# ethnhe/FFB6D

Measured on AMD Instinct MI355X. Metric: RGB-D frames/sec fwd (480x640, N=12288, bs=8), higher is better.
Workload: dtype f32; 1 GPU; FFB6D forward incl. on-device 22-call KNN index pyramid; bs=8/GPU, N=12288 pts, 480x640 RGB-D, 22 classes, fp32, eval; global_batch=8, n_points=12288, index_dtype=int64, layout=pm, parallelism=dp1 (independent batches, one process per GPU, no process group)

## Files before the change

### ffb6d_amd/_lib.py

```python
import ctypes
import os

from . import build as _build

_c = ctypes
_vp, _i64, _i32, _sz = _c.c_void_p, _c.c_int64, _c.c_int, _c.c_size_t

SIGNATURES = {
    "ffb6d_last_error": (_c.c_char_p, []),
    "ffb6d_abi_version": (_c.c_int, []),
    "cpp_knn": (None, [_vp, _sz, _sz, _vp, _sz, _sz, _vp]),
    "cpp_knn_omp": (None, [_vp, _sz, _sz, _vp, _sz, _sz, _vp]),
    "cpp_knn_batch": (None, [_vp, _sz, _sz, _sz, _vp, _sz, _sz, _vp]),
    "cpp_knn_batch_omp": (None, [_vp, _sz, _sz, _sz, _vp, _sz, _sz, _vp]),
    "cpp_knn_batch_distance_pick": (None, [_vp, _sz, _sz, _sz, _vp, _sz, _sz, _vp]),
    "cpp_knn_batch_distance_pick_omp": (None, [_vp, _sz, _sz, _sz, _vp, _sz, _sz, _vp]),
    "ffb6d_knn_workspace_bytes": (_sz, [_i64, _i64, _i64, _i32]),
    "ffb6d_knn_batch_device": (_i32, [_vp, _vp, _i64, _i64, _i64, _i32, _vp, _vp, _vp, _vp, _sz, _vp]),
    "ffb6d_knn_prepared_bytes": (_sz, [_i64, _i64]),
    "ffb6d_knn_prepare_workspace_bytes": (_sz, [_i64, _i64]),
    "ffb6d_knn_prepare": (_i32, [_vp, _i64, _i64, _vp, _sz, _vp, _sz, _vp]),
    "ffb6d_knn_prepare_multi_workspace_bytes": (_sz, [_i32, _vp, _i64]),
    "ffb6d_knn_prepare_multi": (_i32, [_i32, _vp, _vp, _i64, _vp, _vp, _vp, _sz, _vp]),
    "ffb6d_knn_search_multi": (_i32, [_i32, _vp, _i64, _vp]),
    "ffb6d_knn_search_prepared": (_i32, [_vp, _vp, _vp, _i64, _i64, _i64, _i32, _vp, _vp, _vp, _vp]),
    "ffb6d_knn_set_pair_counter": (_i32, [_vp]),
    "ffb6d_knn_uses_pruning": (_i32, [_i64, _i64, _i64, _i32]),
    "ffb6d_random_sample_f32": (_i32, [_vp, _vp, _i32, _vp, _vp, _i64, _i64, _i64, _i64, _i32, _vp]),
    "ffb6d_random_sample_bwd_f32": (_i32, [_vp, _vp, _vp, _i64, _i64, _i64, _i64, _vp]),
    "ffb6d_nearest_interpolation_f32": (_i32, [_vp, _vp, _i32, _vp, _i64, _i64, _i64, _i64, _vp]),
    "ffb6d_nearest_interpolation_bwd_f32": (_i32, [_vp, _vp, _i32, _vp, _i64, _i64, _i64, _i64, _vp]),
    "ffb6d_gather_neighbour_f32": (_i32, [_vp, _vp, _i32, _vp, _i64, _i64, _i64, _i64, _i32, _vp]),
    "ffb6d_gather_neighbour_bwd_f32": (_i32, [_vp, _vp, _i32, _vp, _i64, _i64, _i64, _i64, _i32, _vp]),
    "ffb6d_relative_pos_encoding_f32": (_i32, [_vp, _vp, _i32, _vp, _i64, _i64, _i32, _vp]),
    "ffb6d_att_pool_f32": (_i32, [_vp, _vp, _vp, _i64, _i64, _i64, _i32, _vp]),
    "ffb6d_relative_pos_encoding_cm_f32": (_i32, [_vp, _vp, _i32, _vp, _i64, _i64, _i32, _vp]),
    "ffb6d_att_pool_bwd_f32": (_i32, [_vp, _vp, _vp, _vp, _vp, _i64, _i64, _i64, _i32, _vp]),
    "ffb6d_mlp_pm_f32": (_i32, [_vp, _vp, _vp, _i64, _i64, _vp, _i64, _vp, _i64, _i64, _vp, _i64, _vp, _i64, _i32, _i64, _vp,
                                _i64, _i64, _i64, _i32, _i32, _vp]),
    "ffb6d_mlp_pm_tile": (_i32, [_i64, _i64, _i64, _i32]),
    "ffb6d_mlp_pm_choice": (_i32, [_i64, _i64, _i64, _i64, _i32, _i32, _i32]),
    "ffb6d_mlp_pm_seq_plan": (_i32, [_i64, _i64]),
    "ffb6d_mlp_pm_batched_f32": (_i32, [_vp, _i64, _i64, _vp, _i64, _i64, _vp, _i64, _i64, _i64, _i32, _vp]),
    "ffb6d_mlp_pm_split_w": (_i32, [_vp, _vp, _i64, _vp]),
    "ffb6d_mlp_pm_split_f32": (_i32, [_vp, _vp, _vp, _i64, _i64, _vp, _i64, _vp, _i64, _i64, _vp, _i64, _vp, _i64, _i32, _i64, _vp,
                                      _i64, _i64, _i64, _i32, _i32, _vp]),
    "ffb6d_mlp_pm_split_batched_f32": (_i32, [_vp, _i64, _i64, _vp, _i64, _i64, _vp, _i64, _i64, _i64, _vp]),
    "ffb6d_wino_input_f32": (_i32, [_vp, _vp, _i64, _i64, _i64, _i64, _i64, _vp]),
    "ffb6d_wino_output_f32": (_i32, [_vp, _vp, _vp, _vp, _vp, _vp, _vp, _i64, _i64, _i64, _i64, _i64, _i32, _c.c_float, _vp]),
    "ffb6d_wino4_input_f32": (_i32, [_vp, _vp, _i64, _i64, _i64, _i64, _i64, _vp]),
    "ffb6d_wino4_output_f32": (_i32, [_vp, _vp, _vp, _vp, _vp, _vp, _vp, _i64, _i64, _i64, _i64, _i64, _i32, _c.c_float, _vp]),
    "ffb6d_wino4_conv_f32": (_i32, [_vp, _vp, _vp, _vp, _vp, _vp, _vp, _vp, _i64, _i64, _i64, _i64, _i64, _i32, _c.c_float, _i32, _vp]),
    "ffb6d_wino4_conv_form": (_i32, [_i64, _i64]),
    "ffb6d_mlp_pm_set_big_form": (None, [_i32]),
    "ffb6d_mlp_pm_set_seq_lin": (None, [_i32]),
    "ffb6d_att_pool_pm_f32": (_i32, [_vp, _vp, _i64, _i64, _vp, _i32, _vp, _i64, _i64, _vp, _i64, _i64, _i64, _i32, _vp]),
    "ffb6d_mlp_pm_bf16": (_i32, [_vp, _vp, _vp, _i64, _i64, _vp, _i64, _vp, _i64, _i64, _vp, _i64, _vp, _i64, _i32, _i64, _vp,
                                 _i64, _i64, _i64, _i32, _i32, _vp]),
    "ffb6d_att_pool_pm_bf16": (_i32, [_vp, _vp, _i64, _i64, _vp, _i32, _vp, _i64, _i64, _vp, _i64, _i64, _i64, _i32, _vp]),
    "ffb6d_random_sample_pm": (_i32, [_i32, _vp, _vp, _i32, _vp, _i64, _i64, _i64, _i64, _i32, _vp]),
    "ffb6d_gather_rows_pm": (_i32, [_i32, _vp, _vp, _i32, _vp, _i64, _i64, _i64, _i64, _vp]),
    "ffb6d_relative_pos_encoding_pm": (_i32, [_i32, _vp, _vp, _i32, _vp, _i64, _i64, _i32, _vp]),
    "ffb6d_affine_act_pm": (_i32, [_i32, _vp, _vp, _vp, _vp, _vp, _vp, _vp, _i64, _i64, _i32, _c.c_float, _vp]),
    "ffb6d_affine_relu_maxpool_pm": (_i32, [_i32, _vp, _vp, _vp, _vp, _i64, _i64, _i64, _i64, _vp]),
    "ffb6d_bilinear_resize_pm": (_i32, [_i32, _vp, _vp, _i64, _i64, _i64, _i64, _i64, _i64, _i32, _vp]),
    "ffb6d_mlp_chain3_pm_f32": (_i32, [_vp, _i64, _vp, _vp, _i32, _vp, _vp, _i32, _vp, _vp, _i32, _vp, _i64, _i64, _i64, _vp]),
    "ffb6d_mlp_chain3_pm_bf16": (_i32, [_vp, _i64, _vp, _vp, _i32, _vp, _vp, _i32, _vp, _vp, _i32, _vp, _i64, _i64, _i64, _vp]),
    "ffb6d_upsampled_patch_rows_pm": (_i32, [_i32, _vp, _vp, _i32, _vp, _i64, _i64, _i64, _i64, _i64, _i64, _i64, _vp]),
    "ffb6d_posenc_mlp_pm": (_i32, [_i32, _vp, _vp, _i32, _vp, _i64, _vp, _i32, _vp, _i64, _i64, _i32, _i64, _vp]),
    "ffb6d_lfa_pm": (_i32, [_i32, _i32, _vp, _i64, _vp, _i32, _vp, _i64, _vp, _i64, _vp, _i32, _vp, _vp, _i32, _vp, _vp, _vp, _i32, _vp, _i64,
                            _i64, _i64, _i32, _i64, _i32, _vp]),
    "ffb6d_lfa_pm_choice": (_i32, [_i64, _i64, _i32]),
    "ffb6d_bilinear_bwd_pm": (_i32, [_i32, _vp, _vp, _i64, _i64, _i64, _i64, _i64, _i64, _vp]),
    "ffb6d_prelu_fwd": (_i32, [_i32, _vp, _vp, _vp, _i64, _vp]),
    "ffb6d_prelu_bwd": (_i32, [_i32, _vp, _vp, _vp, _vp, _vp, _i64, _vp]),
    "ffb6d_gather_sum_rows": (_i32, [_i32, _vp, _i64, _vp, _vp, _vp, _i64, _i64, _vp]),
    "ffb6d_random_sample_rows_bwd": (_i32, [_i32, _vp, _vp, _i32, _vp, _i64, _vp, _i64, _i64, _i64, _i64, _i32, _vp]),
    "ffb6d_att_pool_rows": (_i32, [_i32, _vp, _i64, _vp, _i64, _vp, _i64, _i32, _i64, _vp]),
    "ffb6d_att_pool_rows_bwd": (_i32, [_i32, _vp, _i64, _vp, _i64, _vp, _i64, _vp, _vp, _i64, _i32, _i64, _vp]),
    "ffb6d_log_softmax_rows": (_i32, [_i32, _vp, _vp, _i64, _i64, _vp]),
    "ffb6d_log_softmax_rows_bwd": (_i32, [_i32, _vp, _vp, _vp, _i64, _i64, _vp]),
    "ffb6d_upconv_combine_pm": (_i32, [_i32, _vp, _vp, _c.c_float, _vp, _i64, _i64, _i64, _i64, _i64, _i64, _vp]),
    "ffb6d_upconv_set_form": (None, [_i32]),
    "ffb6d_pose_set_fit_form": (None, [_i32]),
    "ffb6d_pose_set_fit_spread": (None, [_i32]),
    "ffb6d_pose_set_big_form": (None, [_i32]),
    "ffb6d_psp_pool_pm_workspace_bytes": (_sz, [_i64, _i64, _i64, _vp, _i32]),
    "ffb6d_psp_pool_pm": (_i32, [_i32, _vp, _vp, _i64, _i64, _i64, _i64, _vp, _i32, _vp, _sz, _vp]),
    "ffb6d_psp_prior_sum_pm": (_i32, [_i32, _vp, _vp, _i64, _i64, _i64, _i64, _vp, _i32, _vp]),
    "ffb6d_depth_to_cloud_f32": (_i32, [_vp, _vp, _c.c_float, _vp, _i64, _i64, _i64, _vp]),
    "ffb6d_pyramid_sets_f32": (_i32, [_vp, _i64, _i64, _i64, _i64, _i64, _i32, _vp, _vp, _vp, _vp, _i64, _i64, _i32, _vp, _vp, _vp]),
    "ffb6d_sample_points_workspace_bytes": (_sz, [_i64, _i64, _i64]),
    "ffb6d_sample_points_f32": (_i32, [_vp, _c.c_float, _vp, _vp, _i32, _vp, _c.c_uint64, _vp, _vp, _vp, _vp, _i64, _i64, _i64,
                                       _i64, _vp, _sz, _vp]),
    "ffb6d_depth_normal": (_i32, [_vp, _i32, _c.c_double, _c.c_double, _i32, _i32, _i32, _i32, _vp, _i64, _i64, _i64, _vp]),
    "ffb6d_fill_missing_workspace_bytes": (_sz, [_i64, _i64, _i64]),
    "ffb6d_fill_missing_f32": (_i32, [_vp, _c.c_double, _c.c_double, _c.c_float, _vp, _i64, _i64, _i64, _vp, _sz, _vp]),
    "ffb6d_check_index_range": (_i32, [_vp, _i32, _i64, _i64, _vp, _vp]),
    "ffb6d_vote_sets_f32": (_i32, [_vp, _vp, _vp, _i32, _vp, _vp, _vp, _i32, _i32, _i32, _i32, _i64, _vp, _vp, _vp]),
    "ffb6d_mean_shift_workspace_bytes": (_sz, [_i32, _i64]),
    "ffb6d_mean_shift_f32": (_i32, [_vp, _vp, _i32, _i32, _i64, _i64, _c.c_float, _i32, _i32, _vp, _vp, _vp, _vp, _vp,
                                    _sz, _vp]),
    "ffb6d_mean_shift_multi_workspace_bytes": (_sz, [_i32, _i64]),
    "ffb6d_mean_shift_multi_f32": (_i32, [_vp, _vp, _i32, _i32, _i64, _i64, _c.c_float, _i32, _i32, _i32, _i32, _vp, _vp, _vp, _vp,
                                          _vp, _vp, _sz, _vp]),
    "ffb6d_pose_set_converged_out": (None, [_vp]),
    "ffb6d_set_clusters_to_points": (_i32, [_vp, _vp, _vp, _vp, _i32, _i64, _i32, _vp, _vp]),
    "ffb6d_vote_sets_inst_f32": (_i32, [_vp, _vp, _vp, _i32, _vp, _vp, _vp, _vp, _i32, _i32, _i32, _i32, _i64, _vp, _vp, _vp]),
    "ffb6d_set_labels_to_points": (_i32, [_vp, _vp, _vp, _vp, _i32, _i64, _i32, _vp, _vp]),
    "ffb6d_refine_mask_by_center": (_i32, [_vp, _vp, _vp, _i32, _vp, _vp, _vp, _vp, _i32, _i32, _vp, _vp]),
    "ffb6d_best_fit_transform_f32": (_i32, [_vp, _vp, _i32, _i32, _vp, _vp]),
    "ffb6d_pose_add_adds_workspace_bytes": (_sz, [_i32, _i64]),
    "ffb6d_pose_add_adds_f32": (_i32, [_vp, _vp, _i32, _vp, _vp, _vp, _i32, _vp, _vp, _vp, _sz, _vp]),
    "ffb6d_icp_prepared_bytes": (_sz, [_i64, _i32]),
    "ffb6d_icp_prepare": (_i32, [_vp, _vp, _i32, _i64, _vp, _sz, _vp]),
    "ffb6d_icp_workspace_bytes": (_sz, [_i32, _i64]),
    "ffb6d_icp_set_form": (None, [_i32]),
# ... 135 lines not shown
```

### ffb6d_amd/forward_pm.py

```python
import torch
import torch.nn.functional as F

from . import _lib, ops, ops_pm, pyramid


def cached(mod, name, sources, build):
    key = tuple((t._version, t.data_ptr(), t.device) for t in sources)
    store = mod.__dict__.setdefault("_pm_cache", {})
    hit = store.get(name)
    if hit is None or hit[0] != key:
        with torch.no_grad():
            hit = (key, build())
        store[name] = hit
    return hit[1]


def _pad_k(w, k_to):
    if w.shape[1] == k_to:
        return w.contiguous()
    out = w.new_zeros(w.shape[0], k_to)
    out[:, :w.shape[1]] = w
    return out


# ... 215 lines not shown
        return False
    cout, cin = c.weight.shape[:2]
    if cin < TRUNK_WINOGRAD_MIN_CIN or cin < 128 or cin % 32 or cout % 4:
        return False
    B, H, W, _ = x.shape
    if m is None:
        m = wino_variant(B, H, W)
    planes, Tp = (m + 2) ** 2, (ops_pm.wino4_tiles if m == 4 else ops_pm.wino_tiles)(B, H, W)[1]
    lim = (1 << 31) - (1 << 20)
    return planes * (Tp + 256) * max(cin, cout) * 4 < lim and B * H * W * max(cin, cout) * 4 < lim and planes * cout * cin * 4 < lim


def conv_wino(x, c, scale, shift, residual=None, res_affine=None, m=None):
    if m is None:
        m = wino_variant(*x.shape[:3])
    x = x if x.is_contiguous() else x.contiguous()
    if m == 4:
        v, u = ops_pm.wino4_input(x), wino4_weights(c)
        if gemm_split_takes(v.shape[0] * v.shape[1], u.shape[1], u.shape[2]):
            mm = ops_pm.mlp_batched(v, u, tile_hint=ops_pm.SPLIT_FORM, w_split=wino4_split_weights(c))
        else:
            mm = ops_pm.mlp_batched(v, u)
        return ops_pm.wino4_output(mm, x.shape[:3], scale, shift, act=ops.ACT_RELU, residual=residual, res_affine=res_affine)
    if m != 2:
        raise ValueError(f"conv_wino: m must be 2, 4 or None, got {m}")
    u = wino_weights(c)
    v = ops_pm.wino_input(x)
    mm = ops_pm.mlp_batched(v, u)
    return ops_pm.wino_output(mm, x.shape[:3], scale, shift, act=ops.ACT_RELU, residual=residual, res_affine=res_affine)


TRUNK_WINOGRAD_FUSED = True
TRUNK_WINOGRAD_FUSED_WIDTHS = frozenset({(64, 64), (128, 128), (128, 256)})


def wino_fused_ok(c, x):
    if not (TRUNK_WINOGRAD and TRUNK_WINOGRAD_FUSED) or x.dtype != torch.float32 or c.weight.dtype != torch.float32:
        return False
    if (c.kernel_size, c.stride, c.padding, c.dilation, c.groups) != ((3, 3), (1, 1), (1, 1), (1, 1), 1) or c.bias is not None \
            or c.padding_mode != "zeros":
        return False
    cout, cin = c.weight.shape[:2]
    if (cin, cout) not in TRUNK_WINOGRAD_FUSED_WIDTHS or cin not in ops_pm.WINO4_CONV_CIN or cout not in ops_pm.WINO4_CONV_COUT:
        return False
    B, H, W, _ = x.shape
    return B * H * W * max(cin, cout) * 4 < (1 << 31) - (1 << 20)


def conv_wino_fused(x, c, scale, shift, residual=None, res_affine=None):
    x = x if x.is_contiguous() else x.contiguous()
    return ops_pm.wino4_conv(x, wino4_weights(c), scale, shift, act=ops.ACT_RELU, residual=residual, res_affine=res_affine)


def trunk_conv_form(c, x):
    if wino_fused_ok(c, x):
        return "fused"
    return "wino" if wino_ok(c, x) else "miopen"


def res_block(rb, x):
    form1 = trunk_conv_form(rb.conv1, x)
    if form1 == "fused":
        y = conv_wino_fused(x, rb.conv1, *ops.bn_fold(rb.bn1))
    elif form1 == "wino":
        y = conv_wino(x, rb.conv1, *ops.bn_fold(rb.bn1))
    else:
        y = ops_pm.affine_act_(conv(x, rb.conv1), *ops.bn_fold(rb.bn1), act=ops.ACT_RELU)
    form2 = trunk_conv_form(rb.conv2, y)
    if form2 == "miopen":
        y = conv(y, rb.conv2)
    res, res_affine = x, None
    if rb.downsample is not None:
        res, res_affine = conv(x, rb.downsample[0]), ops.bn_fold(rb.downsample[1])
    if form2 == "fused":
        return conv_wino_fused(y, rb.conv2, *ops.bn_fold(rb.bn2), residual=res, res_affine=res_affine)
    if form2 == "wino":
        return conv_wino(y, rb.conv2, *ops.bn_fold(rb.bn2), residual=res, res_affine=res_affine)
    return ops_pm.affine_act_(y, *ops.bn_fold(rb.bn2), act=ops.ACT_RELU, residual=res, res_affine=res_affine)


def pyramid_pooling(pp, x):
    B, h, w_, C = x.shape
    sizes = [st[0].output_size[0] for st in pp.stages]
    bw = pp.bottleneck.weight

    def build():
        ch = pp.stages[0][1].weight.shape[0]
        wb = bw.detach().reshape(bw.shape[0], -1)
        prods = [(wb[:, i * ch:(i + 1) * ch] @ st[1].weight.detach().reshape(ch, ch)).contiguous()
                 for i, st in enumerate(pp.stages)]
        return prods, wb[:, len(pp.stages) * ch:].contiguous()
    prods, wx = cached(pp, "fold", [bw] + [st[1].weight for st in pp.stages], build)
    pooled = ops_pm.psp_pool(x, sizes)
    zs, off = [], 0
    for s, wl in zip(sizes, prods):
        zs.append(ops_pm.mlp(pooled[:, off:off + s * s].contiguous(), wl, role="cnn"))
        off += s * s
    prior = ops_pm.psp_prior_sum(torch.cat(zs, dim=1), sizes, (h, w_), dtype=x.dtype)
    wx = cached(pp, "wx%s" % x.dtype, [bw], lambda: wx.to(x.dtype))
    return mlp_long(pp, "wx", [bw], x, wx, pp.bottleneck.bias.detach().float(), ops.ACT_RELU, add=prior, role="cnn")


UPCONV_FOLD = "auto"
UPCONV_FOLD_BF16 = True


# ... 171 lines not shown

def forward(net, inputs, end_points, two_streams=True, taps=None):
    dev = inputs['rgb'].device
    dt = torch.bfloat16 if getattr(net, "precision", "fp32") == "bf16" else torch.float32
    ops_pm.MLP_SEQ_FORM = GEMM_SEQ_FORM
    ops_pm.MLP_BIG_FORM = GEMM_BIG_FORM
    ops_pm.MLP_SEQ_LIN = (2 if GEMM_SEQ_LIN_ONE else 1) if GEMM_SEQ_LIN else 0
    main = torch.cuda.current_stream(dev)
    side = net._side_stream(dev) if two_streams else main
    if two_streams:
        side.wait_stream(main)

    lazy = 'cld_nei_idx0' not in inputs
    if lazy:
        inputs = StreamedPyramid(net, inputs, main, side)

    def need(i, up=False):
        if lazy:
            (inputs.up_level if up else inputs.level)(i, side)
            if not two_streams:
                return
            (inputs.up_level if up else inputs.level)(i, main)

    def need_nearest():
        if lazy:
            inputs.nearest(side)
            if two_streams:
                inputs.nearest(main)

    def on_side():
        return torch.cuda.stream(side)

    probe = getattr(net, "_stall_probe", None)

    def handover(t, producer, consumer, tag=None):
        if producer is not consumer:
            ev = torch.cuda.Event()
            ev.record(producer)
            if probe is not None:
                a = torch.cuda.Event(enable_timing=True)
                a.record(consumer)
            consumer.wait_event(ev)
            if probe is not None:
                b = torch.cuda.Event(enable_timing=True)
                b.record(consumer)
                probe.append((tag, a, b))
            t.record_stream(consumer)
        return t

    def fuse(i, pre_p2r, fuse_p2r, pre_r2p, fuse_r2p, rgb0, p0, p2r_idx, r2p_idx):
        st = ("ds%d" if pre_p2r is net.ds_fuse_p2r_pre_layers else "up%d") % i
        return fusion_step(pre_p2r[i], fuse_p2r[i], pre_r2p[i], fuse_r2p[i], rgb0, p0, p2r_idx, r2p_idx, main, side, handover, st)

    rgb = inputs['rgb'].to(dt).contiguous(memory_format=torch.channels_last).permute(0, 2, 3, 1)
    pool = net.cnn_pre_stages[3]
    if STEM_FUSED and (pool.kernel_size, pool.stride, pool.padding, pool.dilation, pool.ceil_mode) == (3, 2, 1, 1, False):
        rgb_emb = ops_pm.affine_relu_maxpool(conv(rgb, net.cnn_pre_stages[0]), *ops.bn_fold(net.cnn_pre_stages[1]))
    else:
        y = ops_pm.affine_act_(conv(rgb, net.cnn_pre_stages[0]), *ops.bn_fold(net.cnn_pre_stages[1]), act=ops.ACT_RELU)
        rgb_emb = pool(y.permute(0, 3, 1, 2)).permute(0, 2, 3, 1)
    with on_side():
        raw = inputs['cld_rgb_nrm']
        x0 = torch.zeros(raw.shape[0], raw.shape[2], (raw.shape[1] + 15) // 16 * 16, dtype=dt, device=dev)
        x0[..., :raw.shape[1]] = raw.transpose(1, 2)
        c_pre = net.rndla_pre_stages.conv.weight.shape[0]
        p_emb = torch.zeros(raw.shape[0], raw.shape[2], (c_pre + 15) // 16 * 16, dtype=dt, device=dev)
        mlp(net.rndla_pre_stages, x0, pad_k=x0.shape[-1], out=p_emb[..., :c_pre])

    ds_emb = []
    for i in range(4):
        rgb0 = cnn_stage(net.cnn_ds_stages[i], rgb_emb)
        need(i)
        with on_side():
            xyz = inputs['cld_xyz%d' % i]
            if LFA_FUSED:
                xyz = inputs.xyz_table(i) if lazy else ops_pm.xyz_table(xyz)
            f_enc = dilated_res_block(net.rndla_ds_stages[i], p_emb, xyz, inputs['cld_nei_idx%d' % i])
            p0 = ops_pm.random_sample(f_enc, inputs['cld_sub_idx%d' % i])
        if i == 0:
            ds_emb.append(f_enc)
        need_nearest()
        rgb_emb, p_emb = fuse(i, net.ds_fuse_p2r_pre_layers, net.ds_fuse_p2r_fuse_layers, net.ds_fuse_r2p_pre_layers,
                              net.ds_fuse_r2p_fuse_layers, rgb0, p0, inputs['p2r_ds_nei_idx%d' % i],
                              inputs['r2p_ds_nei_idx%d' % i])
        ds_emb.append(p_emb)
        if taps is not None:
            torch.cuda.synchronize(dev)
            taps['rgb_emb_ds%d' % i], taps['p_emb_ds%d' % i] = rgb_emb.permute(0, 3, 1, 2).float(), p_emb.transpose(1, 2).unsqueeze(3).float()

    n_up = len(net.rndla_up_stages)
    for i in range(n_up - 1):
        rgb0 = cnn_stage(net.cnn_up_stages[i], rgb_emb)
        need(i, up=True)
        need_nearest()
        with on_side():
            p0 = decode(net.rndla_up_stages[i], ds_emb[-i - 2], p_emb, inputs['cld_interp_idx%d' % (n_up - i - 1)])
        rgb_emb, p_emb = fuse(i, net.up_fuse_p2r_pre_layers, net.up_fuse_p2r_fuse_layers, net.up_fuse_r2p_pre_layers,
                              net.up_fuse_r2p_fuse_layers, rgb0, p0, inputs['p2r_up_nei_idx%d' % i],
                              inputs['r2p_up_nei_idx%d' % i])
        if taps is not None:
            torch.cuda.synchronize(dev)
            taps['rgb_emb_up%d' % i], taps['p_emb_up%d' % i] = rgb_emb.permute(0, 3, 1, 2).float(), p_emb.transpose(1, 2).unsqueeze(3).float()
    B = rgb_emb.shape[0]
    choose = inputs['choose'].reshape(B, -1)
    img = last_stage_at_chosen(net.cnn_up_stages[n_up - 1], rgb_emb, choose) if LAST_STAGE_AT_CHOSEN else None
    if img is not None:
        choose = None
    else:
        rgb_emb = cnn_stage(net.cnn_up_stages[n_up - 1], rgb_emb)
        img = rgb_emb.view(B, -1, rgb_emb.shape[-1])
    with on_side():
        p_emb = decode(net.rndla_up_stages[n_up - 1], ds_emb[0], p_emb, inputs['cld_interp_idx0'])
    handover(p_emb, side, main, "main waits for the last decoder")
# ... 57 lines not shown
```

### ffb6d_amd/ops_pm.py

```python
import torch

from . import _lib
from .ops import ACT_LEAKY, ACT_NONE, ACT_RELU, _idx, _need_gpu, _stream


def _dt(*ts):
    dts = {t.dtype for t in ts if t is not None}
    if len(dts) != 1 or next(iter(dts)) not in (torch.float32, torch.bfloat16):
        raise TypeError(f"row operands must all be float32 or all bfloat16, got {sorted(map(str, dts))}")
    return 1 if next(iter(dts)) == torch.bfloat16 else 0


def rows_view(x):
    C = x.shape[-1]
    x2 = x.reshape(-1, C)
    if x2.stride(1) != 1 or x2.data_ptr() % 16 or (x2.shape[0] > 1 and (x2.stride(0) * x2.element_size()) % 16):
        x2 = x2.contiguous()
    return x2, (x2.stride(0) if x2.shape[0] > 1 else C)


ACT_LOG_SOFTMAX = 3
MLP_SEQ_FORM = True
MLP_BIG_FORM = True
MLP_SEQ_LIN = 0
# ... 450 lines not shown
    ib = bits // 8
    ref_bytes = (12 * B * N + ib * B * N * K + 40 * B * N * K if mode == 1 else 0) + (esz * B * N * h + ib * B * N * K + esz * B * N * K * h) \
        + (2 * esz * B * N * K * d + esz * B * N * d)
    with torch.cuda.device(f.device), _lib.traced("lfa_pm", nbytes, (mode, d, N, dt, flops, ref_bytes)):
        rc = lib.ffb6d_lfa_pm(dt, int(mode), x.data_ptr(), xfs, idx.data_ptr(), bits, f2.data_ptr(), ldf, w1.data_ptr(), w1.stride(0),
                              b1.data_ptr(), int(act1), w2.data_ptr() if w2 is not None else None,
                              b2.data_ptr() if b2 is not None else None, int(act2), wfc.data_ptr(), wm.data_ptr(), bm.data_ptr(),
                              int(actm), out.data_ptr(), out.stride(-2), B, N, K, d, int(p_hint), _stream(f))
    _lib.check(rc, "ffb6d_lfa_pm")
    return out


def affine_act_(x, scale, shift, act=ACT_NONE, slope=0.0, residual=None, res_affine=None):
    _need_gpu(x)
    lib = _lib.load()
    if not x.is_contiguous():
        raise ValueError("affine_act_ needs a contiguous tensor")
    dt = _dt(x, residual)
    C = x.shape[-1]
    rows = x.numel() // C
    r = rs = rb = None
    if residual is not None:
        r = residual if residual.is_contiguous() else residual.contiguous()
        if r.shape != x.shape:
            raise ValueError("residual shape mismatch")
        if res_affine is not None:
            rs, rb = res_affine
    nbytes = x.element_size() * x.numel() * (3 if r is not None else 2)
    with torch.cuda.device(x.device), _lib.traced("affine_act_pm", nbytes, (C, rows)):
        rc = lib.ffb6d_affine_act_pm(dt, x.data_ptr(), scale.data_ptr(), shift.data_ptr(),
                                         r.data_ptr() if r is not None else None,
                                         rs.data_ptr() if rs is not None else None,
                                         rb.data_ptr() if rb is not None else None,
                                         x.data_ptr(), rows, C, int(act), float(slope), _stream(x))
    _lib.check(rc, "ffb6d_affine_act_pm_f32")
    return x


def affine_relu_maxpool(x, scale, shift):
    _need_gpu(x)
    lib = _lib.load()
    xc = x.detach()
    xc = xc if xc.is_contiguous() else xc.contiguous()
    B, H, W, C = xc.shape
    out = torch.empty((B, (H - 1) // 2 + 1, (W - 1) // 2 + 1, C), dtype=x.dtype, device=x.device)
    nbytes = x.element_size() * (xc.numel() + out.numel())
    with torch.cuda.device(x.device), _lib.traced("affine_relu_maxpool_pm", nbytes, (C, H, W)):
        rc = lib.ffb6d_affine_relu_maxpool_pm(_dt(xc), xc.data_ptr(), scale.data_ptr(), shift.data_ptr(), out.data_ptr(), B, H, W, C,
                                              _stream(xc))
    _lib.check(rc, "ffb6d_affine_relu_maxpool_pm")
    return out


def bilinear_resize(x, size, align_corners):
    _need_gpu(x)
    lib = _lib.load()
    xc = x.detach()
    xc = xc if xc.is_contiguous() else xc.contiguous()
    B, IH, IW, C = xc.shape
    OH, OW = int(size[0]), int(size[1])
    out = torch.empty((B, OH, OW, C), dtype=x.dtype, device=x.device)
    nbytes = x.element_size() * B * C * (IH * IW + OH * OW)
    with torch.cuda.device(x.device), _lib.traced("bilinear_resize_pm", nbytes, (C, OH, OW)):
        rc = lib.ffb6d_bilinear_resize_pm(_dt(xc), xc.data_ptr(), out.data_ptr(), B, IH, IW, OH, OW, C,
                                              1 if align_corners else 0, _stream(xc))
    _lib.check(rc, "ffb6d_bilinear_resize_pm_f32")
    return out


def upsampled_patch_rows(x, idx, size):
    _need_gpu(x, idx)
    lib = _lib.load()
    xc = x.detach()
    xc = xc if xc.is_contiguous() else xc.contiguous()
    B, IH, IW, C = xc.shape
    if idx.dim() != 2 or idx.shape[0] != B:
        raise ValueError("idx must be [B,P]")
    P = idx.shape[1]
    ii, bits = _idx(idx.reshape(-1))
    OH, OW = int(size[0]), int(size[1])
    out = torch.empty((B, P, 9 * C), dtype=x.dtype, device=x.device)
    nbytes = x.element_size() * B * C * (IH * IW + 9 * P) + B * P * (bits // 8)
    with torch.cuda.device(x.device), _lib.traced("upsampled_patch_rows_pm", nbytes, (C, OH, OW, P)):
        rc = lib.ffb6d_upsampled_patch_rows_pm(_dt(xc), xc.data_ptr(), ii.data_ptr(), bits, out.data_ptr(), B, IH, IW, OH, OW, C, P,
                                               _stream(xc))
    _lib.check(rc, "ffb6d_upsampled_patch_rows_pm")
    return out


def upconv_combine(z, shift, slope, size):
    _need_gpu(z)
    lib = _lib.load()
    zc = z.detach()
    zc = zc if zc.is_contiguous() else zc.contiguous()
    B, IH, IW, C9 = zc.shape
    if C9 % 9 or shift.dtype != torch.float32 or shift.numel() * 9 != C9 or not shift.is_contiguous():
        raise ValueError(f"z {tuple(z.shape)} must hold 9 tap blocks of the {shift.numel()} channels of a contiguous float32 shift")
    C = C9 // 9
    OH, OW = int(size[0]), int(size[1])
    out = torch.empty((B, OH, OW, C), dtype=z.dtype, device=z.device)
    nbytes = z.element_size() * (zc.numel() + out.numel())
    with torch.cuda.device(z.device), _lib.traced("upconv_combine_pm", nbytes, (C, OH, OW)):
        rc = lib.ffb6d_upconv_combine_pm(_dt(zc), zc.data_ptr(), shift.data_ptr(), float(slope), out.data_ptr(), B, IH, IW, OH, OW,
                                         C, _stream(zc))
    _lib.check(rc, "ffb6d_upconv_combine_pm")
    return out
# ... 38 lines not shown
```

### include/ffb6d_ops.h

```cpp
#ifndef FFB6D_OPS_H_
#define FFB6D_OPS_H_

#include "ffb6d_knn.h"

#ifdef __cplusplus
extern "C" {
#endif

int ffb6d_random_sample_f32(const float* feat, const void* idx, int idx_bits,
                            float* out, int32_t* arg,
                            int64_t B, int64_t C, int64_t M, int64_t Np, int K,
                            ffb6d_stream_t stream);

int ffb6d_random_sample_bwd_f32(const float* grad_out, const int32_t* arg, float* grad_feat,
                                int64_t B, int64_t C, int64_t M, int64_t Np,
                                ffb6d_stream_t stream);

int ffb6d_nearest_interpolation_f32(const float* feat, const void* idx, int idx_bits,
                                    float* out,
                                    int64_t B, int64_t C, int64_t M, int64_t U,
                                    ffb6d_stream_t stream);

int ffb6d_nearest_interpolation_bwd_f32(const float* grad_out, const void* idx, int idx_bits,
                                        float* grad_feat,
// ... 47 lines not shown
int ffb6d_mlp_pm_seq_plan(int64_t rows, int64_t cout);
void ffb6d_mlp_pm_set_seq_lin(int on);
void ffb6d_mlp_pm_set_big_form(int on);

int ffb6d_mlp_pm_batched_f32(const float* w, int64_t w_stride, int64_t rows_per_w, const float* x, int64_t k, int64_t ld, float* out,
                             int64_t ldo, int64_t rows, int64_t cout, int tile_hint, ffb6d_stream_t stream);

int ffb6d_mlp_pm_split_w(const float* w, void* w3, int64_t n, ffb6d_stream_t stream);
int ffb6d_mlp_pm_split_f32(const void* w3, const float* bias, const float* x1, int64_t k1, int64_t ld1, const void* x1_idx,
                           int64_t x1_rows_per_frame, const float* x2, int64_t k2, int64_t ld2, const float* y, int64_t ldy,
                           const void* y_idx, int64_t y_rows_per_frame, int idx_bits, int64_t rows_per_frame, float* out, int64_t ldo,
                           int64_t rows, int64_t cout, int act, int variant, ffb6d_stream_t stream);
int ffb6d_mlp_pm_split_batched_f32(const void* w3, int64_t n_w, int64_t rows_per_w, const float* x, int64_t k, int64_t ld, float* out,
                                   int64_t ldo, int64_t rows, int64_t cout, ffb6d_stream_t stream);

int ffb6d_wino_input_f32(const float* x, float* v, int64_t B, int64_t H, int64_t W, int64_t C, int64_t Tp, ffb6d_stream_t stream);
int ffb6d_wino_output_f32(const float* m, const float* scale, const float* shift, const float* res, const float* rscale,
                          const float* rshift, float* out, int64_t B, int64_t H, int64_t W, int64_t O, int64_t Tp, int act, float slope,
                          ffb6d_stream_t stream);

int ffb6d_wino4_input_f32(const float* x, float* v, int64_t B, int64_t H, int64_t W, int64_t C, int64_t Tp, ffb6d_stream_t stream);
int ffb6d_wino4_output_f32(const float* m, const float* scale, const float* shift, const float* res, const float* rscale,
                           const float* rshift, float* out, int64_t B, int64_t H, int64_t W, int64_t O, int64_t Tp, int act, float slope,
                           ffb6d_stream_t stream);

int ffb6d_wino4_conv_f32(const float* x, const float* u, const float* scale, const float* shift, const float* res, const float* rscale,
                         const float* rshift, float* out, int64_t B, int64_t H, int64_t W, int64_t C, int64_t O, int act, float slope,
                         int form, ffb6d_stream_t stream);
int ffb6d_wino4_conv_form(int64_t C, int64_t O);

int ffb6d_att_pool_pm_f32(const float* w_fc, const float* f, int64_t c1, int64_t ldf, const void* nei, int idx_bits,
                          const float* g, int64_t c2, int64_t ldg, float* out, int64_t ldo, int64_t B, int64_t N, int K,
                          ffb6d_stream_t stream);

int ffb6d_mlp_pm_bf16(const void* w, const float* bias, const void* x1, int64_t k1, int64_t ld1, const void* x1_idx,
                      int64_t x1_rows_per_frame, const void* x2, int64_t k2, int64_t ld2, const void* y, int64_t ldy,
                      const void* y_idx, int64_t y_rows_per_frame, int idx_bits, int64_t rows_per_frame, void* out,
                      int64_t ldo, int64_t rows, int64_t cout, int act, int tile_hint, ffb6d_stream_t stream);
int ffb6d_att_pool_pm_bf16(const void* w_fc, const void* f, int64_t c1, int64_t ldf, const void* nei, int idx_bits,
                           const void* g, int64_t c2, int64_t ldg, void* out, int64_t ldo, int64_t B, int64_t N, int K,
                           ffb6d_stream_t stream);

int ffb6d_random_sample_pm(int dtype, const void* feat, const void* idx, int idx_bits, void* out, int64_t B, int64_t M,
                           int64_t C, int64_t Np, int K, ffb6d_stream_t stream);
int ffb6d_gather_rows_pm(int dtype, const void* feat, const void* idx, int idx_bits, void* out, int64_t B, int64_t M,
                         int64_t C, int64_t U, ffb6d_stream_t stream);
int ffb6d_relative_pos_encoding_pm(int dtype, const float* xyz, const void* idx, int idx_bits, void* out, int64_t B,
                                   int64_t N, int K, ffb6d_stream_t stream);
int ffb6d_affine_act_pm(int dtype, const void* x, const float* scale, const float* shift, const void* res,
                        const float* rscale, const float* rshift, void* out, int64_t rows, int64_t C, int act, float slope,
                        ffb6d_stream_t stream);
int ffb6d_affine_relu_maxpool_pm(int dtype, const void* x, const float* scale, const float* shift, void* out, int64_t B, int64_t IH,
                                 int64_t IW, int64_t C, ffb6d_stream_t stream);
int ffb6d_bilinear_resize_pm(int dtype, const void* in, void* out, int64_t B, int64_t IH, int64_t IW, int64_t OH, int64_t OW,
                             int64_t C, int align_corners, ffb6d_stream_t stream);
int ffb6d_mlp_chain3_pm_f32(const float* x, int64_t ldx, const float* w1k, const float* b1, int act1, const float* w2k, const float* b2,
                            int act2, const float* w3k, const float* b3, int act3, float* out, int64_t ldo, int64_t rows, int64_t cout3,
                            ffb6d_stream_t stream);
int ffb6d_mlp_chain3_pm_bf16(const void* x, int64_t ldx, const void* w1k, const float* b1, int act1, const void* w2k, const float* b2,
                             int act2, const void* w3k, const float* b3, int act3, void* out, int64_t ldo, int64_t rows, int64_t cout3,
                             ffb6d_stream_t stream);
int ffb6d_upsampled_patch_rows_pm(int dtype, const void* in, const void* idx, int idx_bits, void* out, int64_t B, int64_t IH,
                                  int64_t IW, int64_t OH, int64_t OW, int64_t C, int64_t P, ffb6d_stream_t stream);
int ffb6d_posenc_mlp_pm(int dtype, const float* xyz, const void* idx, int idx_bits, const float* w, int64_t ldw, const float* bias,
                        int act, void* out, int64_t B, int64_t N, int K, int64_t cout, ffb6d_stream_t stream);
int ffb6d_lfa_pm(int dtype, int mode, const float* xyz4, int64_t xyz_frame_stride, const void* nei, int idx_bits, const void* f, int64_t ldf,
                 const float* w1, int64_t ldw1, const float* b1, int act1, const void* w2, const float* b2, int act2,
                 const void* wfc, const void* wm_kc, const float* bm, int actm, void* out, int64_t ldo, int64_t B, int64_t N,
                 int K, int64_t d, int p_hint, ffb6d_stream_t stream);
int ffb6d_lfa_pm_choice(int64_t npts, int64_t d, int bf16);
int ffb6d_bilinear_bwd_pm(int dtype, const void* grad_out, void* grad_in, int64_t B, int64_t IH, int64_t IW, int64_t OH, int64_t OW,
                          int64_t C, ffb6d_stream_t stream);
int ffb6d_prelu_fwd(int dtype, const void* x, const float* slope, void* y, int64_t n, ffb6d_stream_t stream);
int ffb6d_prelu_bwd(int dtype, const void* x, const void* grad_out, const float* slope, void* grad_x, float* grad_slope, int64_t n,
                    ffb6d_stream_t stream);

int ffb6d_gather_sum_rows(int dtype, const void* g, int64_t ldg, const int64_t* order, const int64_t* start, void* out, int64_t R,
                          int64_t C, ffb6d_stream_t stream);
int ffb6d_random_sample_rows_bwd(int dtype, const void* feat, const void* idx, int idx_bits, const void* g, int64_t ldg, float* acc,
                                 int64_t B, int64_t M, int64_t C, int64_t Np, int K, ffb6d_stream_t stream);
int ffb6d_att_pool_rows(int dtype, const void* feat, int64_t ldf, const void* scores, int64_t lds, void* out, int64_t P, int K,
                        int64_t C, ffb6d_stream_t stream);
int ffb6d_att_pool_rows_bwd(int dtype, const void* g, int64_t ldg, const void* feat, int64_t ldf, const void* scores, int64_t lds,
                            void* gfeat, void* gscores, int64_t P, int K, int64_t C, ffb6d_stream_t stream);
int ffb6d_log_softmax_rows(int dtype, const void* x, void* y, int64_t R, int64_t C, ffb6d_stream_t stream);
int ffb6d_log_softmax_rows_bwd(int dtype, const void* g, const void* x, void* gx, int64_t R, int64_t C, ffb6d_stream_t stream);
int ffb6d_upconv_combine_pm(int dtype, const void* z, const float* shift, float slope, void* out, int64_t B, int64_t IH,
                            int64_t IW, int64_t OH, int64_t OW, int64_t C, ffb6d_stream_t stream);
void ffb6d_upconv_set_form(int form);
size_t ffb6d_psp_pool_pm_workspace_bytes(int64_t B, int64_t H, int64_t C, const int* sizes, int nsizes);
int ffb6d_psp_pool_pm(int dtype, const void* x, float* out, int64_t B, int64_t H, int64_t W, int64_t C, const int* sizes,
                      int nsizes, void* workspace, size_t workspace_bytes, ffb6d_stream_t stream);
int ffb6d_psp_prior_sum_pm(int dtype, const float* z, void* out, int64_t B, int64_t H, int64_t W, int64_t M, const int* sizes,
                           int nsizes, ffb6d_stream_t stream);

int ffb6d_depth_to_cloud_f32(const float* depth, const double* K, float cam_scale, float* out,
                             int64_t B, int64_t H, int64_t W, ffb6d_stream_t stream);

int ffb6d_pyramid_sets_f32(const float* cloud, int64_t cloud_frame_stride, int64_t cloud_coord_stride, int64_t cloud_point_stride,
                           int64_t B, int64_t N, int n_levels, const int64_t* level_n, float* const* level_out, float* table,
                           const float* dpt_xyz, int64_t H, int64_t W, int n_grids, const int* strides, float* const* grid_out,
                           ffb6d_stream_t stream);

int ffb6d_check_index_range(const void* idx, int idx_bits, int64_t count, int64_t M,
                            int32_t* bad, ffb6d_stream_t stream);

// ... 5 lines not shown
```

Before: 760.8 frames/s.

## Fuse stem 7x7 conv, BN, ReLU and maxpool into one MFMA kernel

Adds a HIP kernel that computes the stride-2 7x7 stem convolution with fp32 MFMA from an LDS input window, applies the folded BN and ReLU, and max-pools through LDS atomics before writing the pooled NHWC map. It replaces the channels_last copy, the MIOpen conv and a separate affine/relu/maxpool pass. This avoids writing and re-reading the full-resolution 64-channel conv output. In exchange, overlapping halo conv pixels are recomputed per tile and the pooling relies on LDS atomics.

New measurement: 763.7 frames/s (median of 6 runs). About the same (+0.4%).

```diff
diff --git a/ffb6d_amd/_lib.py b/ffb6d_amd/_lib.py
--- a/ffb6d_amd/_lib.py
+++ b/ffb6d_amd/_lib.py
@@ -63,6 +63,7 @@
     "ffb6d_relative_pos_encoding_pm": (_i32, [_i32, _vp, _vp, _i32, _vp, _i64, _i64, _i32, _vp]),
     "ffb6d_affine_act_pm": (_i32, [_i32, _vp, _vp, _vp, _vp, _vp, _vp, _vp, _i64, _i64, _i32, _c.c_float, _vp]),
     "ffb6d_affine_relu_maxpool_pm": (_i32, [_i32, _vp, _vp, _vp, _vp, _i64, _i64, _i64, _i64, _vp]),
+    "ffb6d_stem_conv_pool_f32": (_i32, [_vp, _i64, _i64, _i64, _i64, _vp, _vp, _vp, _vp, _i64, _i64, _i64, _i64, _i64, _vp]),
     "ffb6d_bilinear_resize_pm": (_i32, [_i32, _vp, _vp, _i64, _i64, _i64, _i64, _i64, _i64, _i32, _vp]),
     "ffb6d_mlp_chain3_pm_f32": (_i32, [_vp, _i64, _vp, _vp, _i32, _vp, _vp, _i32, _vp, _vp, _i32, _vp, _i64, _i64, _i64, _vp]),
     "ffb6d_mlp_chain3_pm_bf16": (_i32, [_vp, _i64, _vp, _vp, _i32, _vp, _vp, _i32, _vp, _vp, _i32, _vp, _i64, _i64, _i64, _vp]),
diff --git a/ffb6d_amd/csrc/stem.hip b/ffb6d_amd/csrc/stem.hip
--- /dev/null
+++ b/ffb6d_amd/csrc/stem.hip
@@ -0,0 +1,154 @@
+#include "common.h"
+#include "ffb6d_ops.h"
+#include "mfma_pm.h"
+
+namespace ffb6d {
+namespace stem {
+
+using pm::f32x16;
+using pm::make_rsrc;
+using pm::u32x4;
+
+constexpr int OOB = 0x7ffffff0;
+constexpr int TPH = 8, TPW = 16;
+constexpr int CH = 2 * TPH + 1, CW = 2 * TPW + 1;
+constexpr int NPIX = CH * CW, NMB = (NPIX + 31) / 32;
+constexpr int WH = 2 * (CH - 1) + 7, WW = 2 * (CW - 1) + 7, PLANE = WH * WW;
+constexpr int WIN = 3 * PLANE, WIN_PAD = (WIN + 3) / 4 * 4;
+constexpr int O = 64, K = 147, KS = (K + 1) / 2;
+constexpr int G = 8, NG = (KS + G - 1) / G;
+constexpr int POOL = TPH * TPW * O;
+constexpr int BLK = 256;
+
+struct StemGeom {
+    int H, W, OH, OW, PH, PW;
+    int TH, TW;
+    int sb, sc, sh, sw;
+};
+
+constexpr int koff(int k) { return k < K ? (k / 49) * PLANE + ((k % 49) / 7) * WW + (k % 7) : 0; }
+
+__global__ void __launch_bounds__(BLK, 2)
+stem_conv_pool_f32_kernel(const float* __restrict__ x, const float* __restrict__ wt, const float* __restrict__ scale,
+                          const float* __restrict__ shift, float* __restrict__ out, const StemGeom g, unsigned x_bytes, unsigned o_bytes)
+{
+    __shared__ __attribute__((aligned(16))) unsigned lds[WIN_PAD + POOL];
+    float* const win = reinterpret_cast<float*>(lds);
+    unsigned* const pool = lds + WIN_PAD;
+
+    const int tid = (int)threadIdx.x, lane = tid & 63, wave = __builtin_amdgcn_readfirstlane(tid >> 6);
+    const int j = lane & 31, h = lane >> 5;
+    const int c0 = (wave & 1) * 32;
+    const int tile = (int)blockIdx.x;
+    const int tx = tile % g.TW, ty = (tile / g.TW) % g.TH, b = tile / (g.TW * g.TH);
+    const int py0 = ty * TPH, px0 = tx * TPW;
+    const int cy0 = 2 * py0 - 1, cx0 = 2 * px0 - 1;
+    const int iy0 = 2 * cy0 - 3, ix0 = 2 * cx0 - 3;
+    const __amdgpu_buffer_rsrc_t rs_x = make_rsrc(x, x_bytes), rs_o = make_rsrc(out, o_bytes);
+
+    float wr[KS];
+#pragma unroll
+    for (int s = 0; s < KS; ++s) wr[s] = wt[(2 * s + h) * O + c0 + j];
+    const float sc = scale[c0 + j], sf = shift[c0 + j];
+
+    const bool chan_fast = g.sc < g.sw;
+#pragma unroll 3
+    for (int e = tid; e < WIN; e += BLK) {
+        const int y = e / (3 * WW), r = e - y * (3 * WW);
+        const int c = chan_fast ? r % 3 : r / WW, xx = chan_fast ? r / 3 : r % WW;
+        const int gy = iy0 + y, gx = ix0 + xx;
+        const bool in = gy >= 0 && gy < g.H && gx >= 0 && gx < g.W;
+        const int off = in ? (b * g.sb + c * g.sc + gy * g.sh + gx * g.sw) * 4 : OOB;
+        win[c * PLANE + y * WW + xx] = __uint_as_float(__builtin_amdgcn_raw_buffer_load_b32(rs_x, off, 0, 0));
+    }
+    for (int e = tid; e < POOL / 4; e += BLK) reinterpret_cast<uint4*>(pool)[e] = make_uint4(0u, 0u, 0u, 0u);
+    __syncthreads();
+
+#pragma unroll 1
+    for (int mb = wave >> 1; mb < NMB; mb += 2) {
+        const int ra = mb * 32 + j, ya = ra / CW, xa = ra - ya * CW;
+        const float* const src = win + (ra < NPIX ? 2 * ya * WW + 2 * xa : 0);
+        f32x16 acc = {0.f, 0.f, 0.f, 0.f, 0.f, 0.f, 0.f, 0.f, 0.f, 0.f, 0.f, 0.f, 0.f, 0.f, 0.f, 0.f};
+        float av[2][G];
+        auto read_group = [&](int n, float (&a)[G]) {
+#pragma unroll
+            for (int i = 0; i < G; ++i)
+                if (n * G + i < KS) a[i] = src[h ? koff(2 * (n * G + i) + 1) : koff(2 * (n * G + i))];
+        };
+        read_group(0, av[0]);
+#pragma unroll
+        for (int n = 0; n < NG; ++n) {
+            if (n + 1 < NG) read_group(n + 1, av[(n + 1) & 1]);
+            __builtin_amdgcn_sched_barrier(0);
+#pragma unroll
+            for (int i = 0; i < G; ++i)
+                if (n * G + i < KS) acc = __builtin_amdgcn_mfma_f32_32x32x2f32(av[n & 1][i], wr[n * G + i], acc, 0, 0, 0);
+            __builtin_amdgcn_sched_barrier(0);
+        }
+
+#pragma unroll
+        for (int q = 0; q < 16; ++q) {
+            const int r = mb * 32 + (q & 3) + 8 * (q >> 2) + 4 * h, cy = r / CW, cx = r - cy * CW;
+            const int gy = cy0 + cy, gx = cx0 + cx;
+            if (r >= NPIX || gy < 0 || gy >= g.OH || gx < 0 || gx >= g.OW) continue;
+            float v = fmaf(acc[q], sc, sf);
+            v = !(v <= 0.f) ? v : 0.f;
+            const unsigned bits = __float_as_uint(v);
+            const int p1 = cy >> 1, p0 = p1 - 1 + (cy & 1), q1 = cx >> 1, q0 = q1 - 1 + (cx & 1);
+            unsigned* const dst = pool + c0 + j;
+            if (p1 < TPH) {
+                if (q1 < TPW) __hip_atomic_fetch_max(dst + (p1 * TPW + q1) * O, bits, __ATOMIC_RELAXED, __HIP_MEMORY_SCOPE_WORKGROUP);
+                if (q0 != q1 && q0 >= 0) __hip_atomic_fetch_max(dst + (p1 * TPW + q0) * O, bits, __ATOMIC_RELAXED, __HIP_MEMORY_SCOPE_WORKGROUP);
+            }
+            if (p0 != p1 && p0 >= 0) {
+                if (q1 < TPW) __hip_atomic_fetch_max(dst + (p0 * TPW + q1) * O, bits, __ATOMIC_RELAXED, __HIP_MEMORY_SCOPE_WORKGROUP);
+                if (q0 != q1 && q0 >= 0) __hip_atomic_fetch_max(dst + (p0 * TPW + q0) * O, bits, __ATOMIC_RELAXED, __HIP_MEMORY_SCOPE_WORKGROUP);
+            }
+        }
+    }
+    __syncthreads();
+
+    for (int e = tid; e < POOL / 4; e += BLK) {
+        const int pix = e >> 4, cq = e & 15, py = py0 + pix / TPW, px = px0 + pix % TPW;
+        const int off = (py < g.PH && px < g.PW) ? (((b * g.PH + py) * g.PW + px) * O + cq * 4) * 4 : OOB;
+        const uint4 v = reinterpret_cast<const uint4*>(pool)[e];
+        const u32x4 u = {v.x, v.y, v.z, v.w};
+        __builtin_amdgcn_raw_buffer_store_b128(u, rs_o, off, 0, 0);
+    }
+}
+
+inline bool aligned(const void* p, uintptr_t a) { return (reinterpret_cast<uintptr_t>(p) & (a - 1)) == 0; }
+
+}
+}
+
+extern "C" int ffb6d_stem_conv_pool_f32(const float* x, int64_t sb, int64_t sc, int64_t sh, int64_t sw, const float* wt, const float* scale,
+                                        const float* shift, float* out, int64_t B, int64_t H, int64_t W, int64_t C, int64_t O,
+                                        ffb6d_stream_t stream)
+{
+    using namespace ffb6d;
+    using namespace ffb6d::stem;
+    FFB6D_REQUIRE(B >= 0 && H >= 1 && W >= 1, "stem_conv_pool: bad shape");
+    FFB6D_REQUIRE(C == 3 && O == stem::O, "stem_conv_pool: built for 3 input and 64 output channels (got %lld -> %lld)", (long long)C,
+                  (long long)O);
+    FFB6D_REQUIRE(sb >= 0 && sc >= 1 && sh >= 1 && sw >= 1, "stem_conv_pool: element strides of x must be positive");
+    const int64_t lim = (1LL << 31) - 16;
+    FFB6D_REQUIRE(B < lim && H < (1 << 24) && W < (1 << 24) && sb < lim && sc < lim && sh < lim && sw < lim,
+                  "stem_conv_pool: a tensor of 2 GiB or more (the kernel addresses with 32-bit byte offsets)");
+    const int64_t OH = (H - 1) / 2 + 1, OW = (W - 1) / 2 + 1, PH = (OH - 1) / 2 + 1, PW = (OW - 1) / 2 + 1;
+    const int64_t TH = ceil_div(PH, TPH), TW = ceil_div(PW, TPW);
+    const int64_t x_elems = B ? 1 + (B - 1) * sb + 2 * sc + (H - 1) * sh + (W - 1) * sw : 0;
+    FFB6D_REQUIRE(x_elems * 4 < lim && B * PH * PW * O * 4 < lim && B * TH * TW < lim,
+                  "stem_conv_pool: a tensor of 2 GiB or more (the kernel addresses with 32-bit byte offsets)");
+    if (B == 0) return FFB6D_OK;
+    FFB6D_REQUIRE(x && wt && scale && shift && out, "stem_conv_pool: null pointer");
+    FFB6D_REQUIRE(aligned(x, 4) && aligned(wt, 16) && aligned(scale, 16) && aligned(shift, 16) && aligned(out, 16),
+                  "stem_conv_pool: 16-byte aligned pointers expected (x: 4-byte)");
+    StemGeom g;
+    g.H = (int)H; g.W = (int)W; g.OH = (int)OH; g.OW = (int)OW; g.PH = (int)PH; g.PW = (int)PW; g.TH = (int)TH; g.TW = (int)TW;
+    g.sb = (int)sb; g.sc = (int)sc; g.sh = (int)sh; g.sw = (int)sw;
+    hipLaunchKernelGGL(stem_conv_pool_f32_kernel, dim3((unsigned)(B * TH * TW)), dim3(BLK), 0, as_stream(stream), x, wt, scale, shift, out,
+                       g, (unsigned)(x_elems * 4), (unsigned)(B * PH * PW * O * 4));
+    FFB6D_LAUNCH_CHECK();
+    return FFB6D_OK;
+}
diff --git a/ffb6d_amd/forward_pm.py b/ffb6d_amd/forward_pm.py
--- a/ffb6d_amd/forward_pm.py
+++ b/ffb6d_amd/forward_pm.py
@@ -291,6 +291,33 @@
     return ops_pm.wino4_conv(x, wino4_weights(c), scale, shift, act=ops.ACT_RELU, residual=residual, res_affine=res_affine)
 
 
+STEM_CONV_FUSED = True
+
+
+def stem_conv_fused_ok(c, pool, x, dt):
+    if not STEM_CONV_FUSED or dt != torch.float32 or x.dtype != torch.float32 or c.weight.dtype != torch.float32 or x.dim() != 4:
+        return False
+    if x.device.type != "cuda":
+        return False
+    if torch.is_grad_enabled() and (x.requires_grad or c.weight.requires_grad):
+        return False
+    if (c.kernel_size, c.stride, c.padding, c.dilation, c.groups) != ((7, 7), (2, 2), (3, 3), (1, 1), 1) or c.bias is not None \
+            or c.padding_mode != "zeros" or tuple(c.weight.shape) != (64, 3, 7, 7):
+        return False
+    if (pool.kernel_size, pool.stride, pool.padding, pool.dilation, pool.ceil_mode) != (3, 2, 1, 1, False):
+        return False
+    B, C, H, W = x.shape
+    if C != 3 or min(B, H, W) < 1 or min(x.stride()[1:]) < 1 or x.stride(0) < 0:
+        return False
+    lim = (1 << 31) - (1 << 20)
+    span = 1 + sum((n - 1) * s for n, s in zip(x.shape, x.stride()))
+    return span * 4 < lim and B * (((H - 1) // 2 + 1 - 1) // 2 + 1) * (((W - 1) // 2 + 1 - 1) // 2 + 1) * 64 * 4 < lim
+
+
+def stem_weights(c):
+    return cached(c, "stem_kc", [c.weight], lambda: ops_pm.stem_weight(c.weight))
+
+
 def trunk_conv_form(c, x):
     if wino_fused_ok(c, x):
         return "fused"
@@ -568,13 +595,16 @@
         st = ("ds%d" if pre_p2r is net.ds_fuse_p2r_pre_layers else "up%d") % i
         return fusion_step(pre_p2r[i], fuse_p2r[i], pre_r2p[i], fuse_r2p[i], rgb0, p0, p2r_idx, r2p_idx, main, side, handover, st)
 
-    rgb = inputs['rgb'].to(dt).contiguous(memory_format=torch.channels_last).permute(0, 2, 3, 1)
     pool = net.cnn_pre_stages[3]
-    if STEM_FUSED and (pool.kernel_size, pool.stride, pool.padding, pool.dilation, pool.ceil_mode) == (3, 2, 1, 1, False):
-        rgb_emb = ops_pm.affine_relu_maxpool(conv(rgb, net.cnn_pre_stages[0]), *ops.bn_fold(net.cnn_pre_stages[1]))
+    if stem_conv_fused_ok(net.cnn_pre_stages[0], pool, inputs['rgb'], dt):
+        rgb_emb = ops_pm.stem_conv_pool(inputs['rgb'], stem_weights(net.cnn_pre_stages[0]), *ops.bn_fold(net.cnn_pre_stages[1]))
     else:
-        y = ops_pm.affine_act_(conv(rgb, net.cnn_pre_stages[0]), *ops.bn_fold(net.cnn_pre_stages[1]), act=ops.ACT_RELU)
-        rgb_emb = pool(y.permute(0, 3, 1, 2)).permute(0, 2, 3, 1)
+        rgb = inputs['rgb'].to(dt).contiguous(memory_format=torch.channels_last).permute(0, 2, 3, 1)
+        if STEM_FUSED and (pool.kernel_size, pool.stride, pool.padding, pool.dilation, pool.ceil_mode) == (3, 2, 1, 1, False):
+            rgb_emb = ops_pm.affine_relu_maxpool(conv(rgb, net.cnn_pre_stages[0]), *ops.bn_fold(net.cnn_pre_stages[1]))
+        else:
+            y = ops_pm.affine_act_(conv(rgb, net.cnn_pre_stages[0]), *ops.bn_fold(net.cnn_pre_stages[1]), act=ops.ACT_RELU)
+            rgb_emb = pool(y.permute(0, 3, 1, 2)).permute(0, 2, 3, 1)
     with on_side():
         raw = inputs['cld_rgb_nrm']
         x0 = torch.zeros(raw.shape[0], raw.shape[2], (raw.shape[1] + 15) // 16 * 16, dtype=dt, device=dev)
diff --git a/ffb6d_amd/ops_pm.py b/ffb6d_amd/ops_pm.py
--- a/ffb6d_amd/ops_pm.py
+++ b/ffb6d_amd/ops_pm.py
@@ -526,6 +526,43 @@
     return out
 
 
+STEM_K = 148
+
+
+def stem_weight(w):
+    if w.dtype != torch.float32 or tuple(w.shape) != (64, 3, 7, 7):
+        raise ValueError(f"stem_weight takes a float32 [64, 3, 7, 7] filter, got {w.dtype} {tuple(w.shape)}")
+    wt = w.new_zeros(STEM_K, 64)
+    wt[:147] = w.detach().reshape(64, 147).t()
+    return wt
+
+
+def stem_conv_pool(x, wt, scale, shift, out=None):
+    _need_gpu(x, wt)
+    lib = _lib.load()
+    if x.dtype != torch.float32 or x.dim() != 4:
+        raise ValueError("stem_conv_pool needs a float32 [B,3,H,W] map")
+    x = x.detach()
+    B, C, H, W = x.shape
+    if wt.dtype != torch.float32 or wt.dim() != 2 or wt.shape[0] != STEM_K or not wt.is_contiguous():
+        raise ValueError(f"stem_conv_pool needs the contiguous float32 filter [{STEM_K}, O] of stem_weight, got {tuple(wt.shape)}")
+    O = wt.shape[1]
+    OH, OW = (H - 1) // 2 + 1, (W - 1) // 2 + 1
+    PH, PW = (OH - 1) // 2 + 1, (OW - 1) // 2 + 1
+    if out is None:
+        out = torch.empty(B, PH, PW, O, dtype=torch.float32, device=x.device)
+    if out.shape != (B, PH, PW, O) or not out.is_contiguous() or out.dtype != torch.float32:
+        raise ValueError(f"out must be contiguous float32 [{B}, {PH}, {PW}, {O}]")
+    if scale.dtype != torch.float32 or shift.dtype != torch.float32 or scale.numel() != O or shift.numel() != O:
+        raise ValueError(f"scale and shift must be float32 [{O}]")
+    nbytes = 4 * (x.numel() + wt.numel() + out.numel())
+    with torch.cuda.device(x.device), _lib.traced("stem_conv_pool", nbytes, (B, H, W)):
+        rc = lib.ffb6d_stem_conv_pool_f32(x.data_ptr(), *x.stride(), wt.data_ptr(), scale.data_ptr(), shift.data_ptr(), out.data_ptr(),
+                                          B, H, W, C, O, _stream(x))
+    _lib.check(rc, "ffb6d_stem_conv_pool_f32")
+    return out
+
+
 def bilinear_resize(x, size, align_corners):
     _need_gpu(x)
     lib = _lib.load()
diff --git a/include/ffb6d_ops.h b/include/ffb6d_ops.h
--- a/include/ffb6d_ops.h
+++ b/include/ffb6d_ops.h
@@ -123,6 +123,8 @@
                         ffb6d_stream_t stream);
 int ffb6d_affine_relu_maxpool_pm(int dtype, const void* x, const float* scale, const float* shift, void* out, int64_t B, int64_t IH,
                                  int64_t IW, int64_t C, ffb6d_stream_t stream);
+int ffb6d_stem_conv_pool_f32(const float* x, int64_t sb, int64_t sc, int64_t sh, int64_t sw, const float* wt, const float* scale,
+                             const float* shift, float* out, int64_t B, int64_t H, int64_t W, int64_t C, int64_t O, ffb6d_stream_t stream);
 int ffb6d_bilinear_resize_pm(int dtype, const void* in, void* out, int64_t B, int64_t IH, int64_t IW, int64_t OH, int64_t OW,
                              int64_t C, int align_corners, ffb6d_stream_t stream);
 int ffb6d_mlp_chain3_pm_f32(const float* x, int64_t ldx, const float* w1k, const float* b1, int act1, const float* w2k, const float* b2,
```
